# jhamrick/gaussian_processes

Measured on AMD Instinct MI355X. Metric: GP fit+predict wall-clock (kernel build + Cholesky + solve + log_lh + posterior mean), lower is better.
Workload: dtype f64; 1 GPU; N=65536 d=32 RBF(GaussianKernel) f64, m=1000 test points, h=1 w=0.5*sqrt(d) s=1; N=65536, d=32, m=1000, parallelism=1 GPU

## Files before the change

### gaussian_processes_amd/_lib.py

```python
import ctypes
import os
from ctypes import (POINTER, c_char_p, c_double, c_float, c_int, c_int64, c_size_t,
                    c_uint64, c_void_p)

import numpy as np

_HERE = os.path.dirname(os.path.abspath(__file__))
LIB_PATH = os.path.join(_HERE, "libgpx.so")

OK = 0
ERR_ARG, ERR_HIP, ERR_NO_DEVICE, ERR_NOMEM, ERR_UNSUPPORTED, ERR_INTERNAL = -1, -2, -3, -4, -5, -6
(ROUTE_TRSV_OPS, ROUTE_TRSV_STEPS, ROUTE_PANEL_RES, ROUTE_PANEL_CHAIN, ROUTE_FIT_RIDE, ROUTE_FIT_TWO_SOLVES,
 ROUTE_GEMM_FAST, ROUTE_GEMM_GENERIC, ROUTE_SYRK_EXACT, ROUTE_SYRK_PATCH, ROUTE_MG_BCAST_ONE, ROUTE_MG_BCAST_SAG,
 ROUTE_FIT_OPS_AHEAD, ROUTE_TRSM_OPS, ROUTE_POTRF_PAIR, ROUTE_VAR_CHUNK, ROUTE_LOO_CHUNK, ROUTE_TRSM_L_OPS,
 ROUTE_GRAD_CHUNK, ROUTE_EXTEND, ROUTE_SAMPLE, ROUTE_KAPPLY_FUSED, ROUTE_KAPPLY_GEMM, ROUTE_PATHS_GRAD_CHUNK,
 ROUTE_REMOVE, ROUTE_SPARSE_CHUNK) = range(26)
PROF_RANDN, PROF_RFF, PROF_KAPPLY, PROF_KAPPLY_GRAD, PROF_CHOL_DELETE, PROF_SPARSE_GRAM, PROF_SPARSE_GRAD = 14, 15, 16, 17, 18, 19, 20
F64, F32 = 0, 1
KERNEL_GAUSSIAN, KERNEL_PERIODIC, KERNEL_GAUSSIAN_ARD = 0, 1, 2
ARD_MAX_D = 64
FULL, LOWER = 0, 1
(K, DK_DH, DK_DW, DK_DP, D2K_DHDH, D2K_DHDW, D2K_DHDP, D2K_DWDW, D2K_DWDP, D2K_DPDP) = range(10)
MIN_LOG = -705.6238298100243

MEMBER_BY_NAME = {
    "K": K, "dK_dh": DK_DH, "dK_dw": DK_DW, "dK_dp": DK_DP,
    "d2K_dhdh": D2K_DHDH, "d2K_dhdw": D2K_DHDW, "d2K_dwdh": D2K_DHDW,
    "d2K_dhdp": D2K_DHDP, "d2K_dpdh": D2K_DHDP, "d2K_dwdw": D2K_DWDW,
    "d2K_dwdp": D2K_DWDP, "d2K_dpdw": D2K_DWDP, "d2K_dpdp": D2K_DPDP,
}

MG_ID_BYTES = 128
MG_BCAST_FN = ctypes.CFUNCTYPE(c_int, c_void_p, c_void_p, c_size_t, c_int, c_void_p)
MG_ALLREDUCE_FN = ctypes.CFUNCTYPE(c_int, c_void_p, c_void_p, c_size_t, c_int, c_int, c_void_p)

c_double_p = POINTER(c_double)
c_int_p = POINTER(c_int)

_SIGNATURES = {
    "gpx_version": (c_int, []),
    "gpx_last_error": (c_char_p, []),
    "gpx_device_count": (c_int, [c_int_p]),
    "gpx_set_device": (c_int, [c_int]),
    "gpx_get_device": (c_int, [c_int_p]),
    "gpx_device_info": (c_int, [c_int, c_char_p, c_size_t, c_int_p, c_int_p, POINTER(c_uint64)]),
    "gpx_malloc": (c_int, [POINTER(c_void_p), c_size_t]),
    "gpx_free": (c_int, [c_void_p]),
    "gpx_mem_info": (c_int, [ctypes.POINTER(c_size_t), ctypes.POINTER(c_size_t)]),
    "gpx_memcpy_h2d": (c_int, [c_void_p, c_void_p, c_size_t, c_void_p]),
    "gpx_memcpy_d2h": (c_int, [c_void_p, c_void_p, c_size_t, c_void_p]),
    "gpx_memcpy_d2d": (c_int, [c_void_p, c_void_p, c_size_t, c_void_p]),
    "gpx_memcpy2d_h2d": (c_int, [c_void_p, c_size_t, c_void_p, c_size_t, c_size_t, c_size_t, c_void_p]),
    "gpx_memcpy2d_d2h": (c_int, [c_void_p, c_size_t, c_void_p, c_size_t, c_size_t, c_size_t, c_void_p]),
    "gpx_memset": (c_int, [c_void_p, c_int, c_size_t, c_void_p]),
    "gpx_stream_create": (c_int, [POINTER(c_void_p)]),
    "gpx_stream_destroy": (c_int, [c_void_p]),
    "gpx_stream_sync": (c_int, [c_void_p]),
    "gpx_device_sync": (c_int, []),
    "gpx_event_create": (c_int, [POINTER(c_void_p)]),
    "gpx_event_destroy": (c_int, [c_void_p]),
    "gpx_event_record": (c_int, [c_void_p, c_void_p]),
    "gpx_event_sync": (c_int, [c_void_p]),
    "gpx_event_elapsed_ms": (c_int, [c_void_p, c_void_p, POINTER(c_float)]),
    "gpx_stream_wait_event": (c_int, [c_void_p, c_void_p]),
    "gpx_prof_enable": (c_int, [c_int]),
    "gpx_prof_read": (c_int, [c_int, c_double_p, c_double_p, c_double_p]),
    "gpx_d_kmat": (c_int, [c_int, c_int, c_int, c_void_p, c_int64, c_void_p, c_int64, c_int,
                           c_double_p, c_double, c_int, c_void_p, c_int64, c_void_p]),
    "gpx_d_scale_points": (c_int, [c_int, c_void_p, c_int64, c_int, c_double_p, c_void_p, c_void_p]),
    "gpx_d_mean": (c_int, [c_int, c_int, c_void_p, c_int64, c_void_p, c_int64, c_int, c_double_p,
                           c_void_p, c_void_p, c_void_p]),
    "gpx_d_mean_member": (c_int, [c_int, c_int, c_int, c_void_p, c_int64, c_void_p, c_int64, c_int, c_double_p,
                                  c_void_p, c_void_p, c_void_p]),
    "gpx_d_gemm_nt": (c_int, [c_int, c_int64, c_int64, c_int64, c_double, c_void_p, c_int64,
                              c_void_p, c_int64, c_void_p, c_int64, c_int, c_int64, c_int64,
                              c_void_p]),
    "gpx_d_potrf": (c_int, [c_int, c_void_p, c_int64, c_int64, c_void_p, c_void_p]),
    "gpx_d_potrf_panel": (c_int, [c_int, c_void_p, c_int64, c_int64, c_int64, c_int64, c_int64, c_void_p,
                                  c_void_p]),
    "gpx_d_syrk_bc": (c_int, [c_int, c_int64, c_int64, c_void_p, c_int64, c_int64, c_int64, c_void_p,
                              c_int64, c_int64, c_int64, c_int64, c_int, c_int, c_void_p]),
    "gpx_d_tril": (c_int, [c_int, c_void_p, c_int64, c_int64, c_void_p]),
    "gpx_d_trsv_lower": (c_int, [c_int, c_void_p, c_int64, c_int64, c_void_p, c_void_p, c_int,
                                 c_void_p]),
    "gpx_d_trsv_lower_cols": (c_int, [c_int, c_void_p, c_int64, c_int64, c_int64, c_void_p, c_void_p,
                                      c_void_p]),
    "gpx_d_panel_gemv_t": (c_int, [c_int, c_void_p, c_int64, c_int64, c_int64, c_void_p, c_void_p,
                                   c_void_p, c_void_p]),
    "gpx_d_trsm_right_lt": (c_int, [c_int, c_void_p, c_int64, c_int64, c_void_p, c_int64, c_int64,
                                    c_void_p]),
    "gpx_d_trsm_right_l": (c_int, [c_int, c_void_p, c_int64, c_int64, c_void_p, c_int64, c_int64,
                                   c_void_p]),
    "gpx_d_pred_grad": (c_int, [c_int, c_int, c_void_p, c_int64, c_void_p, c_int64, c_int, c_double_p, c_void_p, c_void_p,
                                c_int64, c_double, c_void_p, c_void_p]),
    "gpx_d_logdet_chol": (c_int, [c_int, c_void_p, c_int64, c_int64, c_void_p, c_void_p]),
    "gpx_d_dot": (c_int, [c_int, c_void_p, c_void_p, c_int64, c_void_p, c_void_p]),
    "gpx_d_var_rows": (c_int, [c_int, c_int, c_void_p, c_int64, c_int64, c_int64, c_void_p, c_int, c_double_p, c_void_p,
                               c_void_p, c_void_p]),
    "gpx_d_loo_rows": (c_int, [c_int, c_void_p, c_int64, c_int64, c_int64, c_int64, c_void_p, c_void_p, c_void_p, c_void_p,
# ... 166 lines not shown

def load():
    global _lib
    if _lib is not None:
        return _lib
    if not os.path.exists(LIB_PATH):
        raise GpxError(
            "libgpx.so not found at %s: build it with `python -c 'import __graft_entry__ as g; "
            "g.build()'` or `make -C gaussian_processes_amd/csrc` -- there is no CPU fallback"
            % LIB_PATH)
    lib = ctypes.CDLL(LIB_PATH, mode=ctypes.RTLD_GLOBAL)
    for name, (res, args) in _SIGNATURES.items():
        fn = getattr(lib, name)
        fn.restype = res
        fn.argtypes = args
    _lib = lib
    return lib


def last_error():
    msg = load().gpx_last_error()
    return msg.decode("utf-8", "replace") if msg else ""


def check(rc):
    if rc == OK:
        return
    msg = last_error() or ("gpx status %d" % rc)
    if rc == ERR_ARG:
        raise ValueError(msg)
    if rc == ERR_NOMEM:
        raise MemoryError(msg)
    if rc == ERR_UNSUPPORTED:
        raise NotImplementedError(msg)
    if rc == ERR_NO_DEVICE:
        raise GpxError("no usable MI355X: " + msg)
    raise GpxError(msg)


def dptr(a):
    return a.ctypes.data_as(c_double_p)


def device_count():
    n = c_int(0)
    check(load().gpx_device_count(ctypes.byref(n)))
    return n.value


def device_info(device=0):
    name = ctypes.create_string_buffer(256)
    cus, mhz, mem = c_int(0), c_int(0), c_uint64(0)
    check(load().gpx_device_info(device, name, 256, ctypes.byref(cus), ctypes.byref(mhz),
                                 ctypes.byref(mem)))
    return {"name": name.value.decode(), "cus": cus.value, "clock_mhz": mhz.value,
            "hbm_bytes": mem.value}


def mem_free():
    f, t = c_size_t(0), c_size_t(0)
    check(load().gpx_mem_info(ctypes.byref(f), ctypes.byref(t)))
    return int(f.value)


def var_plan(dtype_id, n, m, chunk_rows=0, free_bytes=None):
    if free_bytes is None:
        free_bytes = mem_free()
    rows, chunks, nbytes = c_int64(0), c_int64(0), c_size_t(0)
    check(load().gpx_debug_var_plan(int(dtype_id), int(n), int(m), int(chunk_rows), int(free_bytes), ctypes.byref(rows),
                                    ctypes.byref(chunks), ctypes.byref(nbytes)))
    return rows.value, chunks.value, int(nbytes.value)


def route_count(route):
    v = c_int64(0)
    check(load().gpx_debug_route_count(int(route), ctypes.byref(v)))
    return v.value


def route_reset():
    check(load().gpx_debug_route_reset())


def kapply_fused_max(value=-1):
    prev = c_int64(0)
    check(load().gpx_debug_kapply_fused_max(int(value), ctypes.byref(prev)))
    return prev.value


def lapack_info_error(info):
    if info < 0:
        raise GpxError("internal failure inside the factorisation (info = %d)" % info)
    return np.linalg.LinAlgError(
        "%d-th leading minor of the array is not positive definite" % info)
```

### gaussian_processes_amd/csrc/gpx_common.h

```cpp
#pragma once
#include <hip/hip_runtime.h>
#include <stdint.h>
#include <stdio.h>
#include <stdlib.h>
#include <string.h>
#include <math.h>
#include <vector>

#include "../../include/gpx.h"
#include "gpx_tune.h"

namespace gpx {

void set_error(const char *fmt, ...);
int  hip_fail(hipError_t e, const char *what, const char *file, int line);
int  ensure_device();

#define GPX_HIP(call)                                                        \
    do {                                                                     \
        hipError_t e__ = (call);                                             \
        if (e__ != hipSuccess) return gpx::hip_fail(e__, #call, __FILE__, __LINE__); \
    } while (0)

#define GPX_TRY(call)                                                        \
    do {                                                                     \
        int rc__ = (call);                                                   \
        if (rc__ != GPX_OK) return rc__;                                     \
    } while (0)

#define GPX_ARG(cond, msg)                                                   \
    do {                                                                     \
        if (!(cond)) { gpx::set_error("%s: %s", __func__, msg); return GPX_ERR_ARG; } \
    } while (0)

#define GPX_LAUNCH_CHECK()                                                   \
    do {                                                                     \
        hipError_t e__ = hipGetLastError();                                  \
        if (e__ != hipSuccess) return gpx::hip_fail(e__, "kernel launch", __FILE__, __LINE__); \
    } while (0)


enum Route { RT_TRSV_OPS = 0, RT_TRSV_STEPS = 1, RT_PANEL_RES = 2, RT_PANEL_CHAIN = 3, RT_FIT_RIDE = 4,
             RT_FIT_TWO_SOLVES = 5, RT_GEMM_FAST = 6, RT_GEMM_GENERIC = 7, RT_SYRK_EXACT = 8, RT_SYRK_PATCH = 9,
             RT_MG_BCAST_ONE = 10, RT_MG_BCAST_SAG = 11, RT_FIT_OPS_AHEAD = 12, RT_TRSM_OPS = 13, RT_POTRF_PAIR = 14, RT_VAR_CHUNK = 15, RT_LOO_CHUNK = 16,
             RT_TRSM_L_OPS = 17, RT_GRAD_CHUNK = 18, RT_EXTEND = 19, RT_SAMPLE = 20, RT_KAPPLY_FUSED = 21, RT_KAPPLY_GEMM = 22, RT_PATHS_GRAD_CHUNK = 23, RT_REMOVE = 24, RT_SPARSE_CHUNK = 25, RT_COUNT = 26 };
void route_hit(int route);

int check_internal_info(int info);

static inline hipStream_t S(void *s) { return (hipStream_t)s; }
static inline size_t esize(int dtype) { return dtype == GPX_F64 ? 8 : 4; }
static inline int64_t round_up(int64_t v, int64_t m) { return (v + m - 1) / m * m; }
static inline int64_t cdiv(int64_t a, int64_t b) { return (a + b - 1) / b; }

static inline int order(hipEvent_t e, hipStream_t from, hipStream_t to)
{
    GPX_HIP(hipEventRecord(e, from));
    GPX_HIP(hipStreamWaitEvent(to, e, 0));
    return GPX_OK;
}
struct EventPool {
    std::vector<hipEvent_t> ev; size_t next = 0;
    int reserve(size_t count)
    {
        while (ev.size() < count) {
            hipEvent_t x;
            GPX_HIP(hipEventCreateWithFlags(&x, hipEventDisableTiming));
            ev.push_back(x);
        }
        return GPX_OK;
    }
    int get(hipEvent_t *e) { GPX_TRY(reserve(next + 1)); *e = ev[next++]; return GPX_OK; }
    void rewind() { next = 0; }
    void destroy() { for (hipEvent_t e : ev) (void)hipEventDestroy(e); ev.clear(); next = 0; }
    int order(hipStream_t from, hipStream_t to) { hipEvent_t e; GPX_TRY(get(&e)); return gpx::order(e, from, to); }
};

enum ProfClass { PC_KMAT = 0, PC_GEMM = 1, PC_POTRF_DIAG = 2, PC_TRSM_ROWS = 3, PC_TRSV = 4,
                 PC_MEAN = 5, PC_REDUCE = 6, PC_GEMM_SKINNY = 7, PC_GEMM_GENERIC = 8, PC_GEMM_PANEL = 9, PC_GEMM_N64 = 10,
                 PC_TRANSPOSE = 11, PC_PRED_GRAD = 12, PC_EXTEND = 13, PC_RANDN = 14, PC_RFF = 15, PC_KAPPLY = 16, PC_KAPPLY_GRAD = 17, PC_CHOL_DELETE = 18, PC_SPARSE_GRAM = 19, PC_SPARSE_GRAD = 20, PC_COUNT = 21 };
extern bool g_prof_on;
int  prof_begin(int cls, double work, hipStream_t st);
void prof_end(int rec, hipStream_t st);
bool roctx_push(const char *name);
void roctx_pop();
struct RoctxRange {
    bool on;
    explicit RoctxRange(const char *name) : on(roctx_push(name)) {}
    ~RoctxRange() { if (on) roctx_pop(); }
};
const char *prof_class_name(int cls);

extern thread_local int g_prof_mute;
struct ProfScope {
    hipStream_t st; int rec; RoctxRange range;
    ProfScope(int cls, double work, hipStream_t s) : st(s), rec(g_prof_on && g_prof_mute == 0 ? prof_begin(cls, work, s) : -1), range(prof_class_name(cls)) {}
    ~ProfScope() { if (rec >= 0) prof_end(rec, st); }
};

int set_max_lds(const void *fn, int bytes);
constexpr int LDS_CHUNK_MAX = 96 * 1024, LDS_TILE_MAX = 156 * 1024;

struct DeviceGuard {
    int prev = -1; bool switched = false; int rc = GPX_OK;
    explicit DeviceGuard(int device)
    {
        if (hipGetDevice(&prev) != hipSuccess) { (void)hipGetLastError(); prev = -1; }
        if (device >= 0 && device != prev) {
            hipError_t e = hipSetDevice(device);
            if (e != hipSuccess) rc = hip_fail(e, "hipSetDevice", __FILE__, __LINE__);
            else switched = true;
        }
    }
    ~DeviceGuard() { if (switched && prev >= 0) (void)hipSetDevice(prev); }
};

}
#include "gpx_mem.h"
namespace gpx {

struct KParams {
    double c[6];
    double diag_add;
    int kernel;
    int member;
};
int make_kparams(int kernel, int member, const double *params, double diag_add, KParams *out);

// ... 123 lines not shown
```

### gaussian_processes_amd/csrc/gpx_potrf.hip

```cpp
#include "gpx_common.h"
#include "gpx_leaf.h"
#include <vector>

namespace gpx {

constexpr int IBP = IB + 1;


template <typename T, bool INV>
__global__ __launch_bounds__(256) void potrf_diag_kernel(T *__restrict__ blk, int64_t lda, int64_t j0,
                                                         int jb, int *__restrict__ info, T *__restrict__ inv,
                                                         int64_t sblk)
{
    blk += (int64_t)blockIdx.x * sblk;
    info += blockIdx.x;
    if (INV) inv += (int64_t)blockIdx.x * (IB * IB);
    __builtin_amdgcn_s_setprio(3);
    const int tid = threadIdx.x;
    const int tr = tid >> 4, tc = tid & 15;
    __shared__ int s_abort;
    if (tid == 0) s_abort = *info;
    __syncthreads();
    if (s_abort != 0) return;
    T a[4][4];
// ... 49 lines not shown
            for (int e = 0; e < CH; ++e) x[c + e] = v.e[e];
        }
#pragma unroll
        for (int c = 0; c < IB; ++c) {
            T v = x[c];
#pragma unroll
            for (int t = 0; t < c; ++t) v = fma(-x[t], sL[c * IBP + t], v);
            x[c] = v / sL[c * IBP + c];
        }
#pragma unroll
        for (int c = 0; c < IB; c += CH) {
            struct alignas(16) V { T e[CH]; } v;
#pragma unroll
            for (int e = 0; e < CH; ++e) v.e[e] = x[c + e];
            *reinterpret_cast<V *>(xr + c) = v;
        }
    } else {
        for (int c = 0; c < jb; ++c) {
            T v = xr[c];
            for (int t = 0; t < c; ++t) v = fma(-xr[t], sL[c * IBP + t], v);
            xr[c] = v / sL[c * IBP + c];
        }
    }
}

template <typename T>
static int launch_trsm_rows(void *X, int64_t ldx, int64_t rows, const void *Ljj, int64_t ldl, int jb,
                            hipStream_t st, const Batch *bt)
{
    if (rows <= 0 || jb <= 0) return GPX_OK;
    dim3 grid((unsigned)cdiv(rows, 256), (unsigned)(bt ? bt->count : 1)), block(256);
    const int64_t sX = bt ? bt->sA : 0, sL = bt ? bt->sB : 0;
    const bool vec_ok = (jb == IB) && (ldx % (16 / (int64_t)sizeof(T)) == 0) && (((uintptr_t)X) % 16 == 0);
    ProfScope prof(PC_TRSM_ROWS, (double)rows * jb * jb * grid.y, st);
    if (vec_ok)
        hipLaunchKernelGGL((trsm_rows_kernel<T, true>), grid, block, 0, st, (T *)X, ldx, rows,
                           (const T *)Ljj, ldl, jb, sX, sL);
    else
        hipLaunchKernelGGL((trsm_rows_kernel<T, false>), grid, block, 0, st, (T *)X, ldx, rows,
                           (const T *)Ljj, ldl, jb, sX, sL);
    GPX_LAUNCH_CHECK();
    return GPX_OK;
}

int trsm_rows(int dtype, void *X, int64_t ldx, int64_t rows, const void *Ljj, int64_t ldl, int jb,
              hipStream_t st, const Batch *bt)
{
    if (dtype == GPX_F64) return launch_trsm_rows<double>(X, ldx, rows, Ljj, ldl, jb, st, bt);
    return launch_trsm_rows<float>(X, ldx, rows, Ljj, ldl, jb, st, bt);
}

static int64_t outer_block(int64_t n, bool batched = false)
{
    const int64_t forced = tune().potrf_nb;
    if (forced >= IB && forced % IB == 0) return forced;
    if (batched && n >= 8192 && n <= 32768) return 1024;
    if (batched && n >= 4096 && n <= 32768) return 512;
    const long long *thr = tune().potrf_widths;
    if (n <= thr[0]) return 128;
    if (n <= thr[1]) return 256;
    if (n <= thr[2]) return 512;
    return 1024;
}

static thread_local ThreadScratch g_leaf;

template <typename T>
static int potrf_panel_t(T *A, int64_t lda, int64_t n, int64_t r0, int64_t c0, int64_t kb, int *info_dev,
                         hipStream_t st, int dtype, const Batch *bt, int64_t kpre = 0, hipEvent_t done = nullptr,
                         PanelHints hints = {})
{
    const int nbatch = bt ? bt->count : 1;
    const int64_t sM = bt ? bt->sA : 0;
    if (kb % IB == 0 && kb <= panel_res_max()) {
        route_hit(RT_PANEL_RES);
        return potrf_panel_res(dtype, A, lda, n, r0, c0, kb, info_dev, st, bt, kpre, done, hints);
    }
    if (kpre != 0) { set_error("potrf_panel: a folded update needs the resident panel route"); return GPX_ERR_ARG; }
    if (kb <= IB) {
        route_hit(RT_PANEL_CHAIN);
        const int jb = (int)kb;
        T *D = A + r0 * lda + c0;
        const int64_t below = n - (r0 + jb);
        const bool via_inverse = !tune().potrf_trsm_rows && below > 0 && below <= tune().potrf_inv_max &&
                                 jb == IB && lda % (16 / (int64_t)sizeof(T)) == 0 &&
                                 ((uintptr_t)(A + (r0 + jb) * lda + c0)) % 16 == 0;
        T *inv = nullptr;
        if (via_inverse) {
            void *p = nullptr;
            GPX_TRY(g_leaf.get(std::max<size_t>((size_t)nbatch * IB * IB * sizeof(T), IB * IB * 8), &p));
            inv = (T *)p;
        }
        {
            ProfScope prof(PC_POTRF_DIAG, (double)jb * jb * jb / 3.0 * nbatch, st);
            if (inv)
                hipLaunchKernelGGL((potrf_diag_kernel<T, true>), dim3(nbatch), dim3(256), 0, st, D, lda, r0, jb,
                                   info_dev, inv, sM);
            else
                hipLaunchKernelGGL((potrf_diag_kernel<T, false>), dim3(nbatch), dim3(256), 0, st, D, lda, r0, jb,
                                   info_dev, inv, sM);
        }
        GPX_LAUNCH_CHECK();
        if (via_inverse) {
            T *Xb = A + (r0 + jb) * lda + c0;
            Batch bi; bi.count = nbatch; bi.sA = sM; bi.sB = IB * IB; bi.sC = sM;
            GPX_TRY(gemm_nt(dtype, below, jb, jb, Xb, lda, inv, IB, Xb, lda, 1.0, GPX_FULL, 0, 0, st, 1, 0,
                            bt ? &bi : nullptr));
        } else if (below > 0) {
            Batch br; br.count = nbatch; br.sA = sM; br.sB = sM; br.sC = 0;
            GPX_TRY(trsm_rows(dtype, A + (r0 + jb) * lda + c0, lda, below, D, lda, jb, st, bt ? &br : nullptr));
        }
        if (done) GPX_HIP(hipEventRecord(done, st));
        return GPX_OK;
    }
    const int64_t h = ((kb / IB + 1) / 2) * IB;
    GPX_TRY(potrf_panel_t<T>(A, lda, n, r0, c0, h, info_dev, st, dtype, bt, 0, nullptr, hints));
    hints.idle_chip = false;
    T *R = A + (r0 + h) * lda + c0;
    if (panel_res_fold(n - (r0 + h), h, kb - h, sizeof(T), lda, A))
        return potrf_panel_t<T>(A, lda, n, r0 + h, c0 + h, kb - h, info_dev, st, dtype, bt, h, done, hints);
    GPX_TRY(gemm_nt(dtype, n - (r0 + h), kb - h, h, R, lda, R, lda, R + h, lda, -1.0, GPX_LOWER, 0, 0, st, 0, 0, bt));
    return potrf_panel_t<T>(A, lda, n, r0 + h, c0 + h, kb - h, info_dev, st, dtype, bt, 0, done, hints);
}

int potrf_panel(int dtype, void *A, int64_t lda, int64_t n, int64_t r0, int64_t c0, int64_t kb,
                int *info_dev, hipStream_t st, const Batch *bt, int64_t kpre, hipEvent_t done, PanelHints hints)
{
    if (dtype == GPX_F64)
        return potrf_panel_t<double>((double *)A, lda, n, r0, c0, kb, info_dev, st, dtype, bt, kpre, done, hints);
    return potrf_panel_t<float>((float *)A, lda, n, r0, c0, kb, info_dev, st, dtype, bt, kpre, done, hints);
}

struct LookAhead { hipStream_t q = nullptr; EventPool ev; };
static thread_local PerDevice<LookAhead> g_la;

hipStream_t potrf_side_stream()
{
    LookAhead *la = nullptr;
    return g_la.current(&la) == GPX_OK ? la->q : nullptr;
}

static int lookahead_setup(LookAhead **out)
{
    LookAhead *la = nullptr;
    GPX_TRY(g_la.current(&la));
    if (!la->q) {
        int least = 0, greatest = 0;
        GPX_HIP(hipDeviceGetStreamPriorityRange(&least, &greatest));
        GPX_HIP(hipStreamCreateWithPriority(&la->q, hipStreamNonBlocking, greatest));
    }
    la->ev.rewind();
    *out = la;
    return GPX_OK;
}

struct PotrfCtx {
    int dtype; void *A; int64_t n, N, lda; size_t es; int64_t nb; int *info_dev; const Batch *bt;
    hipStream_t st, q;
    EventPool *ev;
    const PotrfHook *hook;
    bool taper;
    char *at(int64_t r, int64_t c) const { return (char *)A + (r * lda + c) * es; }
    int64_t nominal(int64_t k0) const { return (taper && !bt) ? std::min(nb, outer_block(n - k0)) : nb; }
    int update(int64_t row_begin, int64_t c0, int64_t c1, int64_t k0, int64_t depth, int64_t w, hipStream_t s) const
    {
        return syrk_bc(dtype, N, row_begin, A, lda, c0, c1, at(k0, k0), lda, k0, depth, w, 1, 0, s, info_dev, bt);
    }
    int panel(int64_t r, int64_t kb, int64_t kpre, bool idle_chip, hipStream_t s, hipEvent_t *done) const
    {
        GPX_TRY(ev->get(done));
        return potrf_panel(dtype, A, lda, N, r, r, kb, info_dev, s, bt, kpre, *done, PanelHints{idle_chip});
    }
    int progress(int64_t cols_done, hipEvent_t panel_done) const { return hook ? hook->fn(hook->user, cols_done, panel_done) : GPX_OK; }
};

static int potrf_no_lookahead(const PotrfCtx &c)
{
    for (int64_t k0 = 0; k0 < c.n; k0 += c.nb) {
        const int64_t kb = std::min(c.nb, c.n - k0), r = k0 + kb;
        GPX_TRY(potrf_panel(c.dtype, c.A, c.lda, c.N, k0, k0, kb, c.info_dev, c.st, c.bt));
        if (r < c.n) GPX_TRY(c.update(r, r, c.n, k0, kb, c.nb, c.st));
    }
    return GPX_OK;
}

static int potrf_pair_phase(const PotrfCtx &c, int64_t *k0_io, int64_t *kb_io, hipEvent_t *ep_io, hipEvent_t *e_rest)
{
    const int64_t n = c.n;
    const hipStream_t st = c.st, q = c.q;
    const int64_t pair_rows = (c.bt || c.nb != 1024 || c.N - n > 1) ? 0 : tune().pair_rows[c.dtype == GPX_F64 ? 0 : 1];
    auto pair_ok = [&](int64_t k) { return pair_rows > 0 && n - (k + 4 * 1024) >= pair_rows && c.nominal(k + 1024) == 1024 &&
                                           c.nominal(k + 2048) == 1024 && c.nominal(k + 3072) == 1024; };
    int64_t k0 = *k0_io;
    if (*kb_io != 1024 || !pair_ok(k0)) return GPX_OK;
    const int64_t rB = k0 + 1024;
    hipEvent_t epA = *ep_io, epB;
    GPX_HIP(hipStreamWaitEvent(st, epA, 0));
    GPX_TRY(c.update(rB, rB, rB + 1024, k0, 1024, 1024, st));
    GPX_TRY(c.ev->order(st, q));
    GPX_TRY(c.panel(rB, 1024, 0, false, q, &epB));
    GPX_TRY(c.progress(rB, epA));
    route_hit(RT_POTRF_PAIR);
    while (pair_ok(k0)) {
        const int64_t rC = k0 + 2048, rD = rC + 1024, rE = rD + 1024;
        GPX_HIP(hipStreamWaitEvent(st, epB, 0));
        GPX_TRY(c.update(rC, rC, rD, k0, 2048, 1024, st));
        GPX_TRY(c.ev->order(st, q));
        hipEvent_t epC, epD;
        GPX_TRY(c.panel(rC, 1024, 0, false, q, &epC));
        GPX_TRY(c.update(rD, rD, rE, k0, 2048, 1024, st));
        GPX_TRY(c.ev->order(st, q));
        GPX_TRY(gemm_nt(c.dtype, c.N - rD, 1024, 1024, c.at(rD, rC), c.lda, c.at(rD, rC), c.lda, c.at(rD, rD), c.lda, -1.0, GPX_LOWER, rD, rD, q));
        GPX_TRY(c.panel(rD, 1024, 0, false, q, &epD));
        if (rE < n) GPX_TRY(c.update(rE, rE, n, k0, 2048, 1024, st));
        GPX_TRY(c.progress(rC, epB));
        GPX_TRY(c.progress(rD, epC));
        k0 = rC; epA = epC; epB = epD;
    }
    const int64_t rC2 = k0 + 2048;
    GPX_HIP(hipStreamWaitEvent(st, epA, 0));
    if (rC2 < n) GPX_TRY(c.update(rC2, rC2, n, k0, 1024, 1024, st));
    GPX_TRY(c.ev->get(e_rest));
    GPX_HIP(hipEventRecord(*e_rest, st));
    *k0_io = k0 + 1024; *kb_io = 1024; *ep_io = epB;
    return GPX_OK;
}

int potrf(int dtype, void *A, int64_t n, int64_t lda, int *info_dev, hipStream_t st, const Batch *bt, int64_t xrows, bool may_block,
          const PotrfHook *hook)
{
    const int64_t N = n + xrows;
    GPX_HIP(hipMemsetAsync(info_dev, 0, sizeof(int) * (bt ? bt->count : 1), st));
    const int64_t nb = outer_block(n, bt != nullptr);
    if (cdiv(n, nb) <= 1) return potrf_panel(dtype, A, lda, N, 0, 0, n, info_dev, st, bt);
    PotrfCtx c = {dtype, A, n, N, lda, esize(dtype), nb, info_dev, bt, st, nullptr, nullptr, bt ? nullptr : hook,
                  tune().taper != 0 && !tune().potrf_nb_set};
    if (tune().no_lookahead) return potrf_no_lookahead(c);
    LookAhead *la = nullptr;
    GPX_TRY(lookahead_setup(&la));
    const hipStream_t q = c.q = la->q;
    c.ev = &la->ev;
    GPX_TRY(c.ev->order(st, q));
    int64_t k0 = 0, kb = std::min(c.nominal(0), n);
    hipEvent_t ep, e_rest = nullptr;
    GPX_TRY(c.panel(0, kb, 0, !bt, q, &ep));
    bool host_paced = may_block && !bt && n <= tune().host_paced;
    if (host_paced) {
        hipStreamCaptureStatus cs = hipStreamCaptureStatusNone;
        if (hipStreamIsCapturing(st, &cs) != hipSuccess) (void)hipGetLastError();
        else if (cs != hipStreamCaptureStatusNone) host_paced = false;
    }
    GPX_TRY(potrf_pair_phase(c, &k0, &kb, &ep, &e_rest));
    while (true) {
        const int64_t r = k0 + kb;
        GPX_HIP(hipStreamWaitEvent(st, ep, 0));
        if (r >= n) {
            GPX_TRY(c.progress(n, ep));
            break;
        }
        const hipEvent_t ep_k = ep;
        const int64_t w1 = c.nominal(r), kb1 = std::min(w1, n - r);
        const bool fold = panel_res_fold(N - r, kb, kb1, c.es, lda, A);
        hipEvent_t e_gate = nullptr;
        if (!fold) {
            GPX_TRY(c.update(r, r, r + kb1, k0, kb, w1, st));
            GPX_TRY(c.ev->order(st, q));
            if (!bt && N - r <= tune().gate_rows) {
                GPX_TRY(c.ev->get(&e_gate));
                GPX_HIP(hipEventRecord(e_gate, q));
            }
        } else if (e_rest) {
            if (host_paced) GPX_HIP(hipEventSynchronize(e_rest));
            GPX_HIP(hipStreamWaitEvent(q, e_rest, 0));
        }
        const bool idle_chip = !bt && (e_gate != nullptr || (fold && (host_paced || !e_rest)));
        GPX_TRY(c.panel(r, kb1, fold ? kb : 0, idle_chip, q, &ep));
        if (r + kb1 < n) {
            if (e_gate) GPX_HIP(hipStreamWaitEvent(st, e_gate, 0));
            GPX_TRY(c.update(r, r + kb1, n, k0, kb, w1, st));
        }
        GPX_TRY(c.ev->get(&e_rest));
        GPX_HIP(hipEventRecord(e_rest, st));
        GPX_TRY(c.progress(r, ep_k));
        k0 = r; kb = kb1;
    }
    return GPX_OK;
}

}

using namespace gpx;

extern "C" {

int gpx_d_potrf(int dtype, void *A, int64_t n, int64_t lda, int *info_dev, void *stream)
{
    gpx::StreamTurn turn__((hipStream_t)stream);
    GPX_TRY(ensure_device());
    GPX_ARG(dtype == GPX_F64 || dtype == GPX_F32, "dtype must be GPX_F64 or GPX_F32");
    GPX_ARG(n >= 0, "n < 0");
    GPX_ARG(info_dev, "info_dev is NULL");
    if (n == 0) { GPX_HIP(hipMemsetAsync(info_dev, 0, sizeof(int), S(stream))); return GPX_OK; }
    GPX_ARG(A, "A is NULL");
    GPX_ARG(lda >= n, "lda < n");
    GPX_ARG(lda % 16 == 0, "lda must be a multiple of 16 elements");
    GPX_ARG(((uintptr_t)A) % 16 == 0, "A must be 16-byte aligned");
    return potrf(dtype, A, n, lda, info_dev, S(stream));
}

int gpx_d_tril(int dtype, void *A, int64_t n, int64_t lda, void *stream)
{
    GPX_TRY(ensure_device());
    GPX_ARG(dtype == GPX_F64 || dtype == GPX_F32, "dtype must be GPX_F64 or GPX_F32");
    GPX_ARG(n >= 0 && lda >= n, "bad n / lda");
    if (n == 0) return GPX_OK;
    GPX_ARG(A, "A is NULL");
    return tril(dtype, A, n, lda, S(stream));
}

}

extern "C" int gpx_d_potrf_panel(int dtype, void *A, int64_t lda, int64_t n, int64_t r0, int64_t c0,
                                 int64_t kb, int *info_dev, void *stream)
{
    gpx::StreamTurn turn__((hipStream_t)stream);
    GPX_TRY(ensure_device());
    GPX_ARG(dtype == GPX_F64 || dtype == GPX_F32, "dtype must be GPX_F64 or GPX_F32");
    GPX_ARG(n >= 0 && r0 >= 0 && c0 >= 0 && kb >= 0 && r0 + kb <= n, "bad dimensions");
    GPX_ARG(info_dev, "info_dev is NULL");
    if (kb == 0) return GPX_OK;
    GPX_ARG(A, "A is NULL");
    GPX_ARG(lda % 16 == 0 && ((uintptr_t)A) % 16 == 0 && c0 % 16 == 0, "A / lda / c0 must be 16-element aligned");
    return potrf_panel(dtype, A, lda, n, r0, c0, kb, info_dev, S(stream));
}
```

### gaussian_processes_amd/csrc/gpx_tune.h

```cpp
#pragma once
#include <stdint.h>

namespace gpx {

#define GPX_TUNE_LIST(X, XF, XS, X2)                                                                                   \
                                                                               \
    XF(gemm_no_fast, "GPX_GEMM_NO_FAST")                                                                               \
    X(gemm_ablate, "GPX_GEMM_ABLATE", 0)                                                                               \
    X(gemm_pad_lds, "GPX_GEMM_PAD_LDS", 0)                                                                             \
    X(gemm_bn64_tiles, "GPX_GEMM_BN64_TILES", 256)                                                                     \
    X(gemm_exact, "GPX_GEMM_EXACT", 1)                                                                                 \
    X(gemm_fine_tiles, "GPX_GEMM_FINE_TILES", 16384)                                                                   \
    X2(syrk_bn64_tiles, "GPX_SYRK_BN64_TILES", 2600, 4000)                                                             \
                                                              \
    X(fit_ride_max, "GPX_FIT_RIDE_MAX", 16384)                                                                         \
    X(fit_ops_ahead, "GPX_FIT_OPS_AHEAD", 1)                                                                           \
    X(fit_ops_ahead_min, "GPX_FIT_OPS_AHEAD_MIN", 8192)                                                                \
    X(fit_ops_tail, "GPX_FIT_OPS_TAIL", 4)                                                                             \
    XS(batch_max, "GPX_BATCH_MAX", 1)                                                                                  \
    X(io_block_bytes, "GPX_IO_BLOCK_BYTES", (int64_t)64 << 20)                                                         \
    X(kmat_panel_bytes, "GPX_KMAT_PANEL_BYTES", (int64_t)256 << 20)                                                    \
                                                                        \
    XF(force_collectives, "GPX_FORCE_COLLECTIVES")                                                                     \
    X(mg_bcast_chunks, "GPX_MG_BCAST_CHUNKS", 4)                                                                       \
    XF(mg_no_timing, "GPX_MG_NO_TIMING")                                                                               \
    XS(mg_owner_first, "GPX_MG_OWNER_FIRST", 0)                                                                        \
                                                                  \
    XF(trace, "GPX_TRACE")                                                                                             \
    X(potrf_res, "GPX_POTRF_RES", 256)                                                                                 \
    X(res_strict, "GPX_RES_STRICT", 1)                                                                                 \
    X(two_part_rows, "GPX_POTRF_TWO_PART_ROWS", 16384)                                                                 \
    X(two_part_batch, "GPX_POTRF_TWO_PART_BATCH", 98304)                                                               \
    X(leaf_mfma_f32_rows, "GPX_LEAF_MFMA_F32_ROWS", 16384)                                                             \
    X(panel_excl_rows, "GPX_PANEL_EXCL_ROWS", 5120)                                                                    \
    XS(leaf, "GPX_LEAF", 0)                                                                                            \
    X2(leaf4_rows, "GPX_LEAF4_ROWS", 8192, 5120)                                                                       \
    X2(panel_pad_lds, "GPX_PANEL_PAD_LDS", 8 * 1024, 40 * 1024)                                                        \
    X(fold_rows, "GPX_POTRF_FOLD_ROWS", 16384)                                                                         \
    X(fold_k, "GPX_POTRF_FOLD_K", 256)                                                                                 \
                                                                  \
    XS(potrf_nb, "GPX_POTRF_NB", 0)                                                                                    \
    XF(potrf_trsm_rows, "GPX_POTRF_TRSM_ROWS")                                                                         \
    X(potrf_inv_max, "GPX_POTRF_INV_MAX", 16384)                                                                       \
    XF(no_lookahead, "GPX_POTRF_NO_LOOKAHEAD")                                                                         \
    X(taper, "GPX_POTRF_TAPER", 1)                                                                                     \
    X2(pair_rows, "GPX_POTRF_PAIR_ROWS", 0, 0)                                                                         \
    X(host_paced, "GPX_POTRF_HOST_PACED", 16384)                                                                       \
    X(gate_rows, "GPX_POTRF_GATE_ROWS", 16384)                                                                         \
                                                                                 \
    X(trsv_ops, "GPX_TRSV_OPS", 1)                                                                                     \
    X(trsv_ops_min, "GPX_TRSV_OPS_MIN", 10240)                                                                         \
    X(trsm_ops, "GPX_TRSM_OPS", 1)                                                                                     \
                                                                          \
    XF(roctx, "GPX_ROCTX")

constexpr int64_t GPX_KAPPLY_FUSED_MAX_F64 = 32;
constexpr int64_t GPX_KAPPLY_FUSED_MAX_F32 = 8;

struct Tune {
#define GPX_T_X(f, e, d) int64_t f = (d);
#define GPX_T_XF(f, e) bool f = false;
#define GPX_T_XS(f, e, d) int64_t f = (d); bool f##_set = false;
#define GPX_T_X2(f, e, d0, d1) int64_t f[2] = {(d0), (d1)};
    GPX_TUNE_LIST(GPX_T_X, GPX_T_XF, GPX_T_XS, GPX_T_X2)
#undef GPX_T_X
#undef GPX_T_XF
#undef GPX_T_XS
#undef GPX_T_X2
    long long potrf_widths[3] = {1, 8192, 12288};
    bool mg_bcast_set = false, mg_bcast_sag = false;
    char rccl_lib[256] = {0};
    int64_t kapply_fused_max[2] = {GPX_KAPPLY_FUSED_MAX_F64, GPX_KAPPLY_FUSED_MAX_F32};
};

const Tune &tune();
void tune_refresh();
int64_t tune_refresh_count();

}
```

### include/gpx.h

```cpp
#ifndef GPX_H
#define GPX_H

#include <stddef.h>
#include <stdint.h>

#ifdef __cplusplus
extern "C" {
#endif

#define GPX_VERSION 100

#define GPX_OK              0
#define GPX_ERR_ARG        -1
#define GPX_ERR_HIP        -2
#define GPX_ERR_NO_DEVICE  -3
#define GPX_ERR_NOMEM      -4
#define GPX_ERR_UNSUPPORTED -5
#define GPX_ERR_INTERNAL   -6

#define GPX_F64 0
#define GPX_F32 1

#define GPX_KERNEL_GAUSSIAN 0
#define GPX_KERNEL_PERIODIC 1
// ... 17 lines not shown
#define GPX_MIN_LOG (-705.6238298100243)

int         gpx_version(void);
const char *gpx_last_error(void);
int gpx_device_count(int *count);
int gpx_set_device(int device);
int gpx_get_device(int *device);
int gpx_device_info(int device, char *name, size_t name_len, int *cus,
                    int *clock_mhz, uint64_t *hbm_bytes);

int gpx_malloc(void **dptr, size_t bytes);
int gpx_free(void *dptr);
int gpx_mem_info(size_t *free_bytes, size_t *total_bytes);
int gpx_memcpy_h2d(void *dst, const void *src, size_t bytes, void *stream);
int gpx_memcpy_d2h(void *dst, const void *src, size_t bytes, void *stream);
int gpx_memcpy_d2d(void *dst, const void *src, size_t bytes, void *stream);
int gpx_memcpy2d_h2d(void *dst, size_t dpitch, const void *src, size_t spitch,
                     size_t row_bytes, size_t rows, void *stream);
int gpx_memcpy2d_d2h(void *dst, size_t dpitch, const void *src, size_t spitch,
                     size_t row_bytes, size_t rows, void *stream);
int gpx_memset(void *dst, int value, size_t bytes, void *stream);

int gpx_stream_create(void **stream);
int gpx_stream_destroy(void *stream);
int gpx_stream_sync(void *stream);
int gpx_device_sync(void);
int gpx_event_create(void **event);
int gpx_event_destroy(void *event);
int gpx_event_record(void *event, void *stream);
int gpx_event_sync(void *event);
int gpx_event_elapsed_ms(void *start, void *stop, float *ms);
int gpx_stream_wait_event(void *stream, void *event);

#define GPX_PROF_KMAT       0
#define GPX_PROF_GEMM       1
#define GPX_PROF_POTRF_DIAG 2
#define GPX_PROF_TRSM_ROWS  3
#define GPX_PROF_TRSV       4
#define GPX_PROF_MEAN       5
#define GPX_PROF_REDUCE     6
#define GPX_PROF_GEMM_SKINNY  7
#define GPX_PROF_GEMM_GENERIC 8
#define GPX_PROF_GEMM_PANEL   9
#define GPX_PROF_GEMM_N64    10
#define GPX_PROF_TRANSPOSE   11
#define GPX_PROF_PRED_GRAD   12
#define GPX_PROF_EXTEND      13
#define GPX_PROF_RANDN       14
#define GPX_PROF_RFF         15
#define GPX_PROF_KAPPLY      16
#define GPX_PROF_KAPPLY_GRAD 17
#define GPX_PROF_CHOL_DELETE 18
#define GPX_PROF_SPARSE_GRAM 19
#define GPX_PROF_SPARSE_GRAD 20
int gpx_prof_enable(int on);
int gpx_prof_read(int cls, double *launches, double *total_ms, double *total_work);

#define GPX_ROUTE_TRSV_OPS        0
#define GPX_ROUTE_TRSV_STEPS      1
#define GPX_ROUTE_PANEL_RES       2
#define GPX_ROUTE_PANEL_CHAIN     3
#define GPX_ROUTE_FIT_RIDE        4
#define GPX_ROUTE_FIT_TWO_SOLVES  5
#define GPX_ROUTE_GEMM_FAST       6
#define GPX_ROUTE_GEMM_GENERIC    7
#define GPX_ROUTE_SYRK_EXACT      8
#define GPX_ROUTE_SYRK_PATCH      9
#define GPX_ROUTE_MG_BCAST_ONE   10
#define GPX_ROUTE_MG_BCAST_SAG   11
#define GPX_ROUTE_FIT_OPS_AHEAD  12
#define GPX_ROUTE_TRSM_OPS       13
#define GPX_ROUTE_POTRF_PAIR     14
#define GPX_ROUTE_VAR_CHUNK      15
#define GPX_ROUTE_LOO_CHUNK      16
#define GPX_ROUTE_TRSM_L_OPS     17
#define GPX_ROUTE_GRAD_CHUNK     18
#define GPX_ROUTE_EXTEND         19
#define GPX_ROUTE_SAMPLE         20
#define GPX_ROUTE_KAPPLY_FUSED   21
#define GPX_ROUTE_KAPPLY_GEMM    22
#define GPX_ROUTE_PATHS_GRAD_CHUNK 23
#define GPX_ROUTE_REMOVE         24
#define GPX_ROUTE_SPARSE_CHUNK   25
int gpx_debug_route_count(int route, int64_t *count);
int gpx_debug_roctx_ranges(int64_t *count);
int gpx_debug_route_reset(void);
int gpx_debug_tune_refreshes(int64_t *count);
int gpx_debug_kapply_fused_max(int64_t value, int64_t *previous);
int gpx_debug_leaf_selfcheck(int run_now, int *state);


int gpx_d_kmat(int dtype, int kernel, int member, const void *x1, int64_t n,
               const void *x2, int64_t m, int d, const double *params,
               double diag_add, int tri, void *out, int64_t ld, void *stream);

int gpx_d_scale_points(int dtype, const void *x, int64_t n, int d, const double *w_host, void *out, void *stream);

int gpx_d_mean(int dtype, int kernel, const void *xo, int64_t m, const void *x,
               int64_t n, int d, const double *params, const void *alpha,
               void *out, void *stream);

int gpx_d_mean_member(int dtype, int kernel, int member, const void *xo, int64_t m, const void *x,
                      int64_t n, int d, const double *params, const void *alpha, void *out, void *stream);

int gpx_d_pred_grad(int dtype, int kernel, const void *xo, int64_t m, const void *x, int64_t n, int d,
                    const double *params, const void *alpha, const void *B, int64_t ldb, double scale,
                    double *out_dev, void *stream);

int gpx_d_gemm_nt(int dtype, int64_t M, int64_t N, int64_t K, double alpha,
                  const void *A, int64_t lda, const void *B, int64_t ldb, void *C,
                  int64_t ldc, int tri, int64_t row0, int64_t col0, void *stream);

int gpx_d_potrf(int dtype, void *A, int64_t n, int64_t lda, int *info_dev,
                void *stream);

int gpx_d_potrf_panel(int dtype, void *A, int64_t lda, int64_t n, int64_t r0, int64_t c0,
                      int64_t kb, int *info_dev, void *stream);
int gpx_d_syrk_bc(int dtype, int64_t n, int64_t row_begin, void *Cloc, int64_t ldc,
                  int64_t cl0, int64_t cl1, const void *Pb, int64_t ldp, int64_t k0,
                  int64_t kb, int64_t nb, int P, int rank, void *stream);

int gpx_d_tril(int dtype, void *A, int64_t n, int64_t lda, void *stream);

int gpx_d_trsv_lower(int dtype, const void *L, int64_t n, int64_t ldl, void *b,
                     void *x, int transpose, void *stream);

int gpx_d_trsv_lower_cols(int dtype, const void *L, int64_t n, int64_t ldl, int64_t ncols,
                          void *b, void *x, void *stream);
int gpx_d_panel_gemv_t(int dtype, const void *Lp, int64_t ldl, int64_t rows, int64_t ncols,
                       const void *x, void *y, void *work, void *stream);

int gpx_d_trsm_right_lt(int dtype, const void *L, int64_t n, int64_t ldl, void *X,
                        int64_t m, int64_t ldx, void *stream);

int gpx_d_trsm_right_l(int dtype, const void *L, int64_t n, int64_t ldl, void *X,
                       int64_t m, int64_t ldx, void *stream);

int gpx_d_logdet_chol(int dtype, const void *L, int64_t n, int64_t ldl,
                      double *out_dev, void *stream);

int gpx_d_var_rows(int dtype, int kernel, const void *X, int64_t rows, int64_t n, int64_t ldx, const void *xo, int d,
                   const double *params, const double *kdiag_dev, double *out_dev, void *stream);

int gpx_d_loo_rows(int dtype, const void *X, int64_t rows, int64_t n, int64_t ldx, int64_t c0, const void *y, const void *alpha,
                   double *kii_dev, double *mean_dev, double *var_dev, double *logp_dev, void *stream);

int gpx_d_dot(int dtype, const void *a, const void *b, int64_t n, double *out_dev,
              void *stream);

int gpx_d_copy_lower(int dtype, const void *src, int64_t lds, void *dst, int64_t ldd, int64_t n, void *stream);
int gpx_d_schur_lower(int dtype, const void *B, int64_t k, int64_t n, int64_t ldb, void *S, int64_t lds, void *stream);
int gpx_d_chol_delete(int dtype, const void *L, int64_t n, int64_t ldl, const int64_t *idx_host, int64_t k, void *out, int64_t ldo,
                      void *stream);

int gpx_d_randn(int dtype, void *out, int64_t rows, int64_t cols, int64_t ld,
                uint64_t seed, uint64_t stream, uint64_t offset, void *hipstream);

int gpx_d_mvn_sample(int dtype, void *C, int64_t m, int64_t ldc, const void *mean, double jitter, int64_t S,
                     uint64_t seed, uint64_t stream, void *Z, int64_t ldz, void *out, int64_t ldo,
                     int *info_dev, void *hipstream);

int gpx_d_rff_features(int dtype, const void *pts, int64_t m, int d, const double *omega_dev, int64_t F, double scale,
                       void *out, int64_t ld, void *stream);

int gpx_d_rff_features_grad(int dtype, const void *pts, int64_t m, int d, const double *omega_dev, int64_t F, double scale,
                            const double *col_div, void *out, int64_t ld, void *stream);
// ... 171 lines not shown
```

Before: 1.324 s.

## Add two-stream lookahead phase to blocked Cholesky for early wide panels

Adds an initial lookahead phase to the blocked Cholesky. While the trailing matrix is still large, panel factorisation and its strip update run on a second stream, overlapping the main trailing update on the primary stream, with events linking the steps. Control then passes to the existing loop. The phase is on by default for f64 above a row threshold. It also drops the potrf_trsm_rows flag and adds a debug plan export. The cost is extra event and stream coordination, and a risk of ordering bugs.

```diff
diff --git a/gaussian_processes_amd/_lib.py b/gaussian_processes_amd/_lib.py
--- a/gaussian_processes_amd/_lib.py
+++ b/gaussian_processes_amd/_lib.py
@@ -14,7 +14,7 @@
  ROUTE_GEMM_FAST, ROUTE_GEMM_GENERIC, ROUTE_SYRK_EXACT, ROUTE_SYRK_PATCH, ROUTE_MG_BCAST_ONE, ROUTE_MG_BCAST_SAG,
  ROUTE_FIT_OPS_AHEAD, ROUTE_TRSM_OPS, ROUTE_POTRF_PAIR, ROUTE_VAR_CHUNK, ROUTE_LOO_CHUNK, ROUTE_TRSM_L_OPS,
  ROUTE_GRAD_CHUNK, ROUTE_EXTEND, ROUTE_SAMPLE, ROUTE_KAPPLY_FUSED, ROUTE_KAPPLY_GEMM, ROUTE_PATHS_GRAD_CHUNK,
- ROUTE_REMOVE, ROUTE_SPARSE_CHUNK) = range(26)
+ ROUTE_REMOVE, ROUTE_SPARSE_CHUNK, ROUTE_POTRF_AHEAD) = range(27)
 PROF_RANDN, PROF_RFF, PROF_KAPPLY, PROF_KAPPLY_GRAD, PROF_CHOL_DELETE, PROF_SPARSE_GRAM, PROF_SPARSE_GRAD = 14, 15, 16, 17, 18, 19, 20
 F64, F32 = 0, 1
 KERNEL_GAUSSIAN, KERNEL_PERIODIC, KERNEL_GAUSSIAN_ARD = 0, 1, 2
@@ -347,6 +347,23 @@
     check(load().gpx_debug_route_reset())
 
 
+AHEAD_MAIN, AHEAD_STRIP, AHEAD_PANEL, AHEAD_PROGRESS = range(4)
+AHEAD_OP_FIELDS = ("kind", "stream", "row", "c0", "c1", "k0", "depth", "wait", "rec")
+
+
+def potrf_ahead_plan(n, xrows, w, threshold, wide_cols=None):
+    fn = load().gpx_debug_potrf_ahead_plan
+    fn.restype = c_int
+    fn.argtypes = [c_int64, c_int64, c_int64, c_int64, c_int64, POINTER(c_int64), c_int, POINTER(c_int64)]
+    cap = 9 * 4 * (int(n) // max(int(w), 1) + 1)
+    out, hand = (c_int64 * max(cap, 1))(), (c_int64 * 5)()
+    k = fn(int(n), int(xrows), int(w), int(threshold), int(n if wide_cols is None else wide_cols), out, cap, hand)
+    if k < 0:
+        check(k)
+    ops = [dict(zip(AHEAD_OP_FIELDS, out[9 * i:9 * i + 9])) for i in range(k)]
+    return ops, dict(zip(("J", "k0", "kb", "ep", "e_rest"), hand[:5]))
+
+
 def kapply_fused_max(value=-1):
     prev = c_int64(0)
     check(load().gpx_debug_kapply_fused_max(int(value), ctypes.byref(prev)))
diff --git a/gaussian_processes_amd/csrc/gpx_common.h b/gaussian_processes_amd/csrc/gpx_common.h
--- a/gaussian_processes_amd/csrc/gpx_common.h
+++ b/gaussian_processes_amd/csrc/gpx_common.h
@@ -43,7 +43,7 @@
 enum Route { RT_TRSV_OPS = 0, RT_TRSV_STEPS = 1, RT_PANEL_RES = 2, RT_PANEL_CHAIN = 3, RT_FIT_RIDE = 4,
              RT_FIT_TWO_SOLVES = 5, RT_GEMM_FAST = 6, RT_GEMM_GENERIC = 7, RT_SYRK_EXACT = 8, RT_SYRK_PATCH = 9,
              RT_MG_BCAST_ONE = 10, RT_MG_BCAST_SAG = 11, RT_FIT_OPS_AHEAD = 12, RT_TRSM_OPS = 13, RT_POTRF_PAIR = 14, RT_VAR_CHUNK = 15, RT_LOO_CHUNK = 16,
-             RT_TRSM_L_OPS = 17, RT_GRAD_CHUNK = 18, RT_EXTEND = 19, RT_SAMPLE = 20, RT_KAPPLY_FUSED = 21, RT_KAPPLY_GEMM = 22, RT_PATHS_GRAD_CHUNK = 23, RT_REMOVE = 24, RT_SPARSE_CHUNK = 25, RT_COUNT = 26 };
+             RT_TRSM_L_OPS = 17, RT_GRAD_CHUNK = 18, RT_EXTEND = 19, RT_SAMPLE = 20, RT_KAPPLY_FUSED = 21, RT_KAPPLY_GEMM = 22, RT_PATHS_GRAD_CHUNK = 23, RT_REMOVE = 24, RT_SPARSE_CHUNK = 25, RT_POTRF_AHEAD = 26, RT_COUNT = 27 };
 void route_hit(int route);
 
 int check_internal_info(int info);
diff --git a/gaussian_processes_amd/csrc/gpx_potrf.hip b/gaussian_processes_amd/csrc/gpx_potrf.hip
--- a/gaussian_processes_amd/csrc/gpx_potrf.hip
+++ b/gaussian_processes_amd/csrc/gpx_potrf.hip
@@ -155,7 +155,7 @@
         const int jb = (int)kb;
         T *D = A + r0 * lda + c0;
         const int64_t below = n - (r0 + jb);
-        const bool via_inverse = !tune().potrf_trsm_rows && below > 0 && below <= tune().potrf_inv_max &&
+        const bool via_inverse = below > 0 && below <= tune().potrf_inv_max &&
                                  jb == IB && lda % (16 / (int64_t)sizeof(T)) == 0 &&
                                  ((uintptr_t)(A + (r0 + jb) * lda + c0)) % 16 == 0;
         T *inv = nullptr;
@@ -299,6 +299,66 @@
     return GPX_OK;
 }
 
+enum AheadKind { AH_MAIN = 0, AH_STRIP = 1, AH_PANEL = 2, AH_PROGRESS = 3 };
+struct AheadOp {
+    int kind, stream;
+    int64_t row, c0, c1, k0, depth;
+    int wait, rec;
+};
+struct AheadPlan {
+    std::vector<AheadOp> ops;
+    int64_t J = 0;
+    int64_t k0 = 0, kb = 0; int ep = -1, e_rest = -1;
+};
+static void potrf_ahead_plan(int64_t n, int64_t xrows, int64_t w, int64_t threshold, int64_t wide_cols, AheadPlan *p)
+{
+    (void)xrows;
+    *p = AheadPlan{};
+    auto in_phase = [&](int64_t j) { const int64_t r = j * w; return threshold > 0 && r + w <= n && r < wide_cols && n - (r + w) >= threshold; };
+    int64_t J = 0;
+    while (in_phase(J + 1)) ++J;
+    if (J == 0) return;
+    for (int64_t j = 1; j <= J; ++j) {
+        const int64_t r = j * w;
+        const int ep_prev = (int)(2 * (j - 1)), em_prev = ep_prev + 1;
+        const int64_t first = std::min(n, j == J ? r + w : r + 2 * w);
+        p->ops.push_back({AH_MAIN, 0, first, first, n, r - w, w, ep_prev, em_prev});
+        const int64_t k = j >= 2 ? r - 2 * w : r - w;
+        p->ops.push_back({AH_STRIP, 1, r, r, r + w, k, r - k, j >= 3 ? (int)(2 * (j - 3) + 1) : -1, -1});
+        p->ops.push_back({AH_PANEL, 1, r, r, r + w, 0, 0, -1, (int)(2 * j)});
+        p->ops.push_back({AH_PROGRESS, -1, 0, 0, r, 0, 0, ep_prev, -1});
+    }
+    p->J = J; p->k0 = J * w; p->kb = w; p->ep = (int)(2 * J); p->e_rest = (int)(2 * (J - 1) + 1);
+}
+
+static int potrf_ahead_phase(const PotrfCtx &c, int64_t *k0_io, int64_t *kb_io, hipEvent_t *ep_io, hipEvent_t *e_rest)
+{
+    const int di = c.dtype == GPX_F64 ? 0 : 1;
+    const int64_t w = c.nb, thr = (c.bt || tune().pair_rows[di] > 0) ? 0 : tune().ahead_rows[di];
+    if (thr <= 0 || *k0_io != 0 || *kb_io != w) return GPX_OK;
+    int64_t wide = 0;
+    while (wide < c.n && c.nominal(wide) == w) wide += w;
+    AheadPlan p;
+    potrf_ahead_plan(c.n, c.N - c.n, w, thr, wide, &p);
+    if (p.J == 0) return GPX_OK;
+    route_hit(RT_POTRF_AHEAD);
+    std::vector<hipEvent_t> ev((size_t)(2 * p.J + 2), nullptr);
+    ev[0] = *ep_io;
+    for (const AheadOp &o : p.ops) {
+        const hipStream_t s = o.stream == 0 ? c.st : c.q;
+        if (o.kind == AH_PROGRESS) { GPX_TRY(c.progress(o.c1, ev[o.wait])); continue; }
+        if (o.wait >= 0) GPX_HIP(hipStreamWaitEvent(s, ev[o.wait], 0));
+        if (o.kind == AH_PANEL) { GPX_TRY(c.panel(o.row, o.c1 - o.c0, 0, false, s, &ev[o.rec])); continue; }
+        GPX_TRY(c.update(o.row, o.c0, o.c1, o.k0, o.depth, w, s));
+        if (o.rec >= 0) {
+            GPX_TRY(c.ev->get(&ev[o.rec]));
+            GPX_HIP(hipEventRecord(ev[o.rec], s));
+        }
+    }
+    *k0_io = p.k0; *kb_io = p.kb; *ep_io = ev[p.ep]; *e_rest = ev[p.e_rest];
+    return GPX_OK;
+}
+
 int potrf(int dtype, void *A, int64_t n, int64_t lda, int *info_dev, hipStream_t st, const Batch *bt, int64_t xrows, bool may_block,
           const PotrfHook *hook)
 {
@@ -323,6 +383,7 @@
         if (hipStreamIsCapturing(st, &cs) != hipSuccess) (void)hipGetLastError();
         else if (cs != hipStreamCaptureStatusNone) host_paced = false;
     }
+    GPX_TRY(potrf_ahead_phase(c, &k0, &kb, &ep, &e_rest));
     GPX_TRY(potrf_pair_phase(c, &k0, &kb, &ep, &e_rest));
     while (true) {
         const int64_t r = k0 + kb;
@@ -393,6 +454,23 @@
 
 }
 
+extern "C" int gpx_debug_potrf_ahead_plan(int64_t n, int64_t xrows, int64_t w, int64_t threshold, int64_t wide_cols,
+                                          int64_t *out, int cap, int64_t *handover)
+{
+    GPX_ARG(n >= 1 && xrows >= 0 && w >= IB && w % IB == 0 && threshold >= 0 && wide_cols >= 0 && cap >= 0 && (out || cap == 0) && handover,
+            "bad arguments");
+    AheadPlan p;
+    potrf_ahead_plan(n, xrows, w, threshold, wide_cols, &p);
+    if (p.ops.size() * 9 > (size_t)cap) { set_error("gpx_debug_potrf_ahead_plan: out holds %d values, %zu are needed", cap, p.ops.size() * 9); return GPX_ERR_ARG; }
+    int64_t *o = out;
+    for (const AheadOp &a : p.ops) {
+        const int64_t v[9] = {a.kind, a.stream, a.row, a.c0, a.c1, a.k0, a.depth, a.wait, a.rec};
+        for (int i = 0; i < 9; ++i) *o++ = v[i];
+    }
+    handover[0] = p.J; handover[1] = p.k0; handover[2] = p.kb; handover[3] = p.ep; handover[4] = p.e_rest;
+    return (int)p.ops.size();
+}
+
 extern "C" int gpx_d_potrf_panel(int dtype, void *A, int64_t lda, int64_t n, int64_t r0, int64_t c0,
                                  int64_t kb, int *info_dev, void *stream)
 {
diff --git a/gaussian_processes_amd/csrc/gpx_tune.h b/gaussian_processes_amd/csrc/gpx_tune.h
--- a/gaussian_processes_amd/csrc/gpx_tune.h
+++ b/gaussian_processes_amd/csrc/gpx_tune.h
@@ -40,11 +40,11 @@
     X(fold_k, "GPX_POTRF_FOLD_K", 256)                                                                                 \
                                                                   \
     XS(potrf_nb, "GPX_POTRF_NB", 0)                                                                                    \
-    XF(potrf_trsm_rows, "GPX_POTRF_TRSM_ROWS")                                                                         \
     X(potrf_inv_max, "GPX_POTRF_INV_MAX", 16384)                                                                       \
     XF(no_lookahead, "GPX_POTRF_NO_LOOKAHEAD")                                                                         \
     X(taper, "GPX_POTRF_TAPER", 1)                                                                                     \
     X2(pair_rows, "GPX_POTRF_PAIR_ROWS", 0, 0)                                                                         \
+    X2(ahead_rows, "GPX_POTRF_AHEAD_ROWS", 16384, 12288)                                                               \
     X(host_paced, "GPX_POTRF_HOST_PACED", 16384)                                                                       \
     X(gate_rows, "GPX_POTRF_GATE_ROWS", 16384)                                                                         \
                                                                                  \
diff --git a/include/gpx.h b/include/gpx.h
--- a/include/gpx.h
+++ b/include/gpx.h
@@ -123,6 +123,7 @@
 #define GPX_ROUTE_PATHS_GRAD_CHUNK 23
 #define GPX_ROUTE_REMOVE         24
 #define GPX_ROUTE_SPARSE_CHUNK   25
+#define GPX_ROUTE_POTRF_AHEAD    26
 int gpx_debug_route_count(int route, int64_t *count);
 int gpx_debug_roctx_ranges(int64_t *count);
 int gpx_debug_route_reset(void);
```

After: 1.318 s (median of 6 runs). Within noise of the previous version (-0.4%).
